# moss-lab/ScanFold

Hardware: AMD Instinct MI355X
Metric: windows/sec (W=120, step=1, 100 shuffles) (higher is better)
Workload: dtype int32 (int16 LDS storage) energies; f64 partition function

## Files before the change

scanfold_amd/csrc/scanfold_hip.hip:

```cpp
#include <math.h>
#include <stddef.h>
#include <stdio.h>
#include <stdlib.h>
#include <string.h>

#include <algorithm>
#include <map>
#include <string>
#include <vector>

#include "../../include/scanfold_hip_long.h"
#include "sf_launch.h"
#include "sf_energy.h"
#include "sf_mfe_full.hip.h"
#include "sf_mfe_fast.hip.h"
#include "sf_mfe_long.hip.h"
#include "sf_mfe_long_batch.hip.h"
#include "sf_mfe_banded.hip.h"
#include "sf_mfe_banded_batch.hip.h"
#include "sf_pf.hip.h"
#include "sf_pf_long.hip.h"
#include "sf_pf_long_batch.hip.h"
#include "sf_pf_banded.hip.h"
#include "sf_pf_fast.hip.h"
// ... 584 lines not shown
    g.slot[k].src.assign((const unsigned char *)&P, (const unsigned char *)&P + nb);
    if (blob_37c) {
      g.slot[k].src.insert(g.slot[k].src.end(), (const unsigned char *)&P37, (const unsigned char *)&P37 + nb);
      g.slot[k].src.insert(g.slot[k].src.end(), (const unsigned char *)&PdH, (const unsigned char *)&PdH + nb);
    }
    g.slot[k].key = key; g.slot[k].valid = true; g.slot[k].fast_ok = F.fast_ok; g.slot[k].span = g.max_bp_span;
    g.slot[k].temperature = temperature_c;
    g.slot[k].pf_kT = X.kT; g.slot[k].pf_MLbase = X.MLbase; g.slot[k].pf_hp30 = X.hp_init[30];
    hit = k;
  } else if (g.slot[hit].span != g.max_bp_span) {
    HIPCHK(hipDeviceSynchronize());
    HIPCHK(hipMemcpy((char *)g.slot[hit].dP + offsetof(SfDevParams, max_pair_dist), &md, sizeof md, hipMemcpyHostToDevice));
    g.slot[hit].span = g.max_bp_span;
  }
  g.slot[hit].used = g.loads;
  g.cur = hit;
  g.dP = g.slot[hit].dP; g.dX = g.slot[hit].dX; g.dF = g.slot[hit].dF;
  g.fast_ok = g.slot[hit].fast_ok;
  g.temperature = temperature_c;
  g.have_params = true;
  return SF_OK;
}

int sf_mfe_batch_dev(const uint8_t *d_seqs, int n, int W, int32_t *d_out, void *stream) {
  int rc = check_ready();
  if (rc) return rc;
  if (n < 0 || W < 1 || W > SF_MAX_W || (n > 0 && (!d_seqs || !d_out))) return SF_ERR_BAD_ARG;
  return launch_mfe(d_seqs, n, W, d_out, stream ? (hipStream_t)stream : g.stream);
}

int sf_mfe_batch(const uint8_t *seqs, int n, int W, int32_t *out) {
  int rc = check_ready();
  if (rc) return rc;
  if (n < 0 || W < 1 || W > SF_MAX_W || (n > 0 && (!seqs || !out))) return SF_ERR_BAD_ARG;
  if (n == 0) return SF_OK;
  if ((rc = ensure(g.seqs, (size_t)n * W))) return rc;
  if ((rc = ensure(g.energies, (size_t)n * sizeof(int32_t)))) return rc;
  HIPCHK(hipMemcpyAsync(g.seqs.p, seqs, (size_t)n * W, hipMemcpyHostToDevice, g.stream));
  if ((rc = launch_mfe((const uint8_t *)g.seqs.p, n, W, (int32_t *)g.energies.p, g.stream))) return rc;
  HIPCHK(hipMemcpyAsync(out, g.energies.p, (size_t)n * sizeof(int32_t), hipMemcpyDeviceToHost, g.stream));
  HIPCHK(hipStreamSynchronize(g.stream));
  return SF_OK;
}

int sf_mfe_trace_batch(const uint8_t *seqs, int n, int W, int32_t *mfe_out, char *db_out) {
  int rc = check_ready();
  if (rc) return rc;
  if (n < 0 || W < 1 || W > SF_MAX_W || (n > 0 && (!seqs || !db_out))) return SF_ERR_BAD_ARG;
  if (n == 0) return SF_OK;
  if ((rc = ensure(g.seqs, (size_t)n * W))) return rc;
  if ((rc = ensure(g.energies, (size_t)n * sizeof(int32_t)))) return rc;
  if ((rc = ensure(g.db, (size_t)n * (W + 1)))) return rc;
  HIPCHK(hipMemcpyAsync(g.seqs.p, seqs, (size_t)n * W, hipMemcpyHostToDevice, g.stream));
  if ((rc = launch_mfe((const uint8_t *)g.seqs.p, n, W, (int32_t *)g.energies.p, g.stream, 1, (char *)g.db.p)))
    return rc;
  if (mfe_out)
    HIPCHK(hipMemcpyAsync(mfe_out, g.energies.p, (size_t)n * sizeof(int32_t), hipMemcpyDeviceToHost, g.stream));
  HIPCHK(hipMemcpyAsync(db_out, g.db.p, (size_t)n * (W + 1), hipMemcpyDeviceToHost, g.stream));
  return read_status(g.stream, false);
}

int sf_pf_batch(const uint8_t *seqs, int n, int W, double *ens_dG, double *mbd, char *centroid, double *cdist) {
  int rc = check_ready();
  if (rc) return rc;
  if (n < 0 || W < 1 || W > SF_MAX_W || (n > 0 && !seqs)) return SF_ERR_BAD_ARG;
  if (n == 0) return SF_OK;
  if ((rc = ensure(g.seqs, (size_t)n * W))) return rc;
  if ((rc = ensure(g.dbl, (size_t)n * 3 * sizeof(double)))) return rc;
  if ((rc = ensure(g.cen, (size_t)n * (W + 1)))) return rc;
  double *d_dG = (double *)g.dbl.p, *d_mbd = d_dG + n, *d_cd = d_mbd + n;
  HIPCHK(hipMemcpyAsync(g.seqs.p, seqs, (size_t)n * W, hipMemcpyHostToDevice, g.stream));
  if ((rc = launch_pf((const uint8_t *)g.seqs.p, n, 1, W, d_dG, d_mbd, (char *)g.cen.p, d_cd, g.stream))) return rc;
  if ((rc = pf_results_to_host(n, W, ens_dG, mbd, centroid, cdist))) return rc;
  HIPCHK(hipStreamSynchronize(g.stream));
  return SF_OK;
}

static int scan_constraints(const uint8_t *seqs, const char *cons, int n, int W, bool *noncanonical) {
  static const uint8_t can[5][5] = {{0, 0, 0, 0, 0}, {0, 0, 0, 0, 1}, {0, 0, 0, 1, 0}, {0, 0, 1, 0, 1}, {0, 1, 0, 1, 0}};
  std::vector<int> stack((size_t)W + 1);
  *noncanonical = false;
  for (int k = 0; k < n; k++) {
    const char *c = cons + (size_t)k * W;
    const uint8_t *s = seqs + (size_t)k * W;
    int sp = 0;
    for (int i = 0; i < W; i++) {
      if (c[i] == '(') stack[sp++] = i;
      else if (c[i] == ')') {
        if (sp == 0) return SF_ERR_CONSTRAINT;
        const int o = stack[--sp];
        if (!can[sf_encode_nt(s[o])][sf_encode_nt(s[i])]) *noncanonical = true;
      }
    }
    if (sp) return SF_ERR_CONSTRAINT;
  }
  return SF_OK;
}

int sf_fold_constrained(const uint8_t *seqs, int n, int W, const char *cons, const int32_t *sc_stack_dcal, unsigned flags,
                        int32_t *mfe_out, char *db_out, double *ens_dG, double *mbd, char *centroid, double *cdist) {
  int rc = check_ready();
  if (rc) return rc;
  if (n < 0 || W < 1 || W > SF_MAX_W || (n > 0 && !seqs)) return SF_ERR_BAD_ARG;
  if (n == 0) return SF_OK;
  const bool want_mfe = !(flags & SF_FOLD_NO_MFE), want_pf = !(flags & SF_FOLD_NO_PF);
  bool noncanonical = false;
  if (cons && (rc = scan_constraints(seqs, cons, n, W, &noncanonical))) return rc;
  if ((rc = ensure(g.seqs, (size_t)n * W))) return rc;
  HIPCHK(hipMemcpyAsync(g.seqs.p, seqs, (size_t)n * W, hipMemcpyHostToDevice, g.stream));
  const char *d_cons = nullptr;
  const int32_t *d_sc = nullptr;
  if (cons) {
    if ((rc = ensure(g.cons, (size_t)n * W))) return rc;
    HIPCHK(hipMemcpyAsync(g.cons.p, cons, (size_t)n * W, hipMemcpyHostToDevice, g.stream));
    d_cons = (const char *)g.cons.p;
  }
  if (sc_stack_dcal) {
    if ((rc = ensure(g.sc, (size_t)n * W * sizeof(int32_t)))) return rc;
    HIPCHK(hipMemcpyAsync(g.sc.p, sc_stack_dcal, (size_t)n * W * sizeof(int32_t), hipMemcpyHostToDevice, g.stream));
    d_sc = (const int32_t *)g.sc.p;
  }
  if (want_mfe) {
    if ((rc = ensure(g.energies, (size_t)n * sizeof(int32_t)))) return rc;
    if ((rc = ensure(g.db, (size_t)n * (W + 1)))) return rc;
    rc = launch_mfe((const uint8_t *)g.seqs.p, n, W, (int32_t *)g.energies.p, g.stream, 1, (char *)g.db.p, d_cons, d_sc, noncanonical);
    if (rc) return rc;
    if (mfe_out)
      HIPCHK(hipMemcpyAsync(mfe_out, g.energies.p, (size_t)n * sizeof(int32_t), hipMemcpyDeviceToHost, g.stream));
    if (db_out) HIPCHK(hipMemcpyAsync(db_out, g.db.p, (size_t)n * (W + 1), hipMemcpyDeviceToHost, g.stream));
  }
  if (want_pf) {
    if ((rc = ensure(g.dbl, (size_t)n * 3 * sizeof(double)))) return rc;
    if ((rc = ensure(g.cen, (size_t)n * (W + 1)))) return rc;
    double *d_dG = (double *)g.dbl.p, *d_mbd = d_dG + n, *d_cd = d_mbd + n;
    if ((rc = launch_pf((const uint8_t *)g.seqs.p, n, 1, W, d_dG, d_mbd, (char *)g.cen.p, d_cd, g.stream, d_cons, noncanonical)))
      return rc;
    if ((rc = pf_results_to_host(n, W, ens_dG, mbd, centroid, cdist))) return rc;
  }
  return read_status(g.stream, false);
}

static int check_scan_args(int L, int W, int step, int win_begin, int n_win, int r, int kind) {
  if (L < 1 || W < 1 || W > SF_MAX_W || step < 1 || win_begin < 0 || n_win < 0 || r < 0) return SF_ERR_BAD_ARG;
  if (kind != SF_SHUFFLE_MONO && kind != SF_SHUFFLE_DI) return SF_ERR_BAD_ARG;
  if (n_win > 0 && (long long)(win_begin + n_win - 1) * step + W > L) return SF_ERR_BAD_ARG;
  return SF_OK;
}

static int launch_shuffle(const uint8_t *d_tr, int L, int W, int step, int win_begin, int n_win, int r, int kind,
                          uint64_t seed, uint8_t *d_seqs, hipStream_t st) {
  const long long total = (long long)n_win * (r + 1);
  if (total <= 0) return SF_OK;
  const int grid = (int)((total + SF_SHUF_BLOCK - 1) / SF_SHUF_BLOCK);
  SF_LAUNCH(sf_shuffle_kernel, grid, SF_SHUF_BLOCK, sf_shuffle_lds_bytes(W), st, d_tr, L, W, step, win_begin, n_win, r, kind, seed, d_seqs);
  HIPCHK(hipGetLastError());
  return SF_OK;
}

int sf_shuffle_windows(const uint8_t *transcript, int L, int W, int step, int win_begin, int n_win, int r, int kind,
                       uint64_t seed, uint8_t *seqs_out) {
  SF_ENTER();
  int rc = check_scan_args(L, W, step, win_begin, n_win, r, kind);
  if (rc) return rc;
  if (!transcript || (n_win > 0 && !seqs_out)) return SF_ERR_BAD_ARG;
  if (n_win == 0) return SF_OK;
  const size_t nb = (size_t)n_win * (r + 1) * W;
  if ((rc = ensure(g.transcript, (size_t)L))) return rc;
  if ((rc = ensure(g.seqs, nb))) return rc;
  HIPCHK(hipMemcpyAsync(g.transcript.p, transcript, (size_t)L, hipMemcpyHostToDevice, g.stream));
  if ((rc = launch_shuffle((const uint8_t *)g.transcript.p, L, W, step, win_begin, n_win, r, kind, seed,
                           (uint8_t *)g.seqs.p, g.stream)))
    return rc;
  HIPCHK(hipMemcpyAsync(seqs_out, g.seqs.p, nb, hipMemcpyDeviceToHost, g.stream));
  HIPCHK(hipStreamSynchronize(g.stream));
  return SF_OK;
}

int sf_scan_dev(const uint8_t *d_tr, int L, int W, int step, int win_begin, int n_win, int r, int kind, uint64_t seed,
                unsigned flags, int32_t *d_energies, char *d_structure, char *d_centroid, double *d_ens_div,
                double *d_ens_dG, void *stream) {
  int rc = check_ready();
  if (rc) return rc;
  if ((rc = check_scan_args(L, W, step, win_begin, n_win, r, kind))) return rc;
  if (!d_tr || (n_win > 0 && !d_energies)) return SF_ERR_BAD_ARG;
  if (n_win == 0) return SF_OK;
  hipStream_t st = stream ? (hipStream_t)stream : g.stream;
  const size_t row_bytes = (size_t)(r + 1) * W;
  int chunk = (int)(((size_t)1 << 30) / row_bytes);
  if (chunk < 1) chunk = 1;
  if (chunk > n_win) chunk = n_win;
  if ((rc = ensure(g.seqs, (size_t)chunk * row_bytes))) return rc;
  uint8_t *d_seqs = (uint8_t *)g.seqs.p;
  for (int w0 = 0; w0 < n_win; w0 += chunk) {
    const int nw = (n_win - w0 < chunk) ? n_win - w0 : chunk;
    if ((rc = launch_shuffle(d_tr, L, W, step, win_begin + w0, nw, r, kind, seed, d_seqs, st))) return rc;
    char *dbp = (!(flags & SF_SCAN_NO_TRACE) && d_structure) ? d_structure + (size_t)w0 * (W + 1) : nullptr;
    if ((rc = launch_mfe(d_seqs, nw * (r + 1), W, d_energies + (size_t)w0 * (r + 1), st, r + 1, dbp))) return rc;
    if (!(flags & SF_SCAN_NO_PF)) {
      if ((rc = launch_pf(d_seqs, nw, r + 1, W, d_ens_dG ? d_ens_dG + w0 : nullptr, d_ens_div ? d_ens_div + w0 : nullptr,
                          d_centroid ? d_centroid + (size_t)w0 * (W + 1) : nullptr, nullptr, st, nullptr, false,
                          d_tr, L, win_begin + w0, step)))
        return rc;
    }
  }
  return SF_OK;
}

int sf_scan(const uint8_t *transcript, int L, int W, int step, int win_begin, int n_win, int r, int kind, uint64_t seed,
            unsigned flags, int32_t *energies, char *structure, char *centroid, double *ens_div, double *ens_dG) {
  int rc = check_ready();
  if (rc) return rc;
  if ((rc = check_scan_args(L, W, step, win_begin, n_win, r, kind))) return rc;
  if (!transcript || (n_win > 0 && !energies)) return SF_ERR_BAD_ARG;
  if (n_win == 0) return SF_OK;
  const size_t ne = (size_t)n_win * (r + 1);
  if ((rc = ensure(g.transcript, (size_t)L))) return rc;
  if ((rc = ensure(g.energies, ne * sizeof(int32_t)))) return rc;
  if ((rc = ensure(g.db, (size_t)n_win * (W + 1)))) return rc;
  if ((rc = ensure(g.cen, (size_t)n_win * (W + 1)))) return rc;
  if ((rc = ensure(g.dbl, (size_t)n_win * 2 * sizeof(double)))) return rc;
  double *d_div = (double *)g.dbl.p, *d_dG = d_div + n_win;
  HIPCHK(hipMemcpyAsync(g.transcript.p, transcript, (size_t)L, hipMemcpyHostToDevice, g.stream));
  rc = sf_scan_dev((const uint8_t *)g.transcript.p, L, W, step, win_begin, n_win, r, kind, seed, flags,
                   (int32_t *)g.energies.p, structure ? (char *)g.db.p : nullptr, centroid ? (char *)g.cen.p : nullptr,
                   ens_div ? d_div : nullptr, ens_dG ? d_dG : nullptr, g.stream);
  if (rc) return rc;
  HIPCHK(hipMemcpyAsync(energies, g.energies.p, ne * sizeof(int32_t), hipMemcpyDeviceToHost, g.stream));
  if (structure && !(flags & SF_SCAN_NO_TRACE))
    HIPCHK(hipMemcpyAsync(structure, g.db.p, (size_t)n_win * (W + 1), hipMemcpyDeviceToHost, g.stream));
  if (!(flags & SF_SCAN_NO_PF)) {
    if (centroid) HIPCHK(hipMemcpyAsync(centroid, g.cen.p, (size_t)n_win * (W + 1), hipMemcpyDeviceToHost, g.stream));
    if (ens_div) HIPCHK(hipMemcpyAsync(ens_div, d_div, n_win * sizeof(double), hipMemcpyDeviceToHost, g.stream));
    if (ens_dG) HIPCHK(hipMemcpyAsync(ens_dG, d_dG, n_win * sizeof(double), hipMemcpyDeviceToHost, g.stream));
  }
  return read_status(g.stream, false);
}

struct TabOut {
  int32_t *gk, *gj, *gcount, *gfirst;
  double *sz, *sm, *se;
};
static TabOut tab_out_views(int64_t n) {
  TabOut o;
  char *p = (char *)g.tab_out.p;
  const size_t n8 = ((size_t)n + 1) & ~(size_t)1;
  o.gk = (int32_t *)p;
  o.gj = o.gk + n8;
  o.gcount = o.gj + n8;
  o.gfirst = o.gcount + n8;
  o.sz = (double *)(o.gfirst + n8);
  o.sm = o.sz + n8;
  o.se = o.sm + n8;
  return o;
}

int sf_tabulate_pairs(const char *structures, int row_stride, int structures_on_device, int n_win, int W,
                      const int32_t *starts, const double *z, const double *mfe, const double *ed, int64_t *n_groups) {
  SF_ENTER();
  g.tab_groups = -1;
  if (n_win < 1 || W < 1 || W > SF_MAX_W || row_stride < W || !structures || !starts || !z || !mfe || !ed || !n_groups)
    return SF_ERR_BAD_ARG;
  for (int w = 1; w < n_win; w++)
    if (starts[w] <= starts[w - 1]) return SF_ERR_TABLE;
  const int64_t span = (int64_t)starts[n_win - 1] + W - starts[0];
  if (span > 0x7fffff00 || (int64_t)n_win * W > 0x7fffff00) return SF_ERR_BAD_ARG;
  const int lo = starts[0], n_coords = (int)span;
  hipStream_t st = g.stream;
  const size_t off_z = (((size_t)n_win * 4) + 7) & ~(size_t)7;
  const size_t off_s = off_z + 3 * (size_t)n_win * 8;
  int rc = ensure(g.tab_in, off_s + (structures_on_device ? 0 : (size_t)n_win * row_stride));
  if (rc) return rc;
  char *in = (char *)g.tab_in.p;
  HIPCHK(hipMemcpyAsync(in, starts, (size_t)n_win * 4, hipMemcpyHostToDevice, st));
  HIPCHK(hipMemcpyAsync(in + off_z, z, (size_t)n_win * 8, hipMemcpyHostToDevice, st));
  HIPCHK(hipMemcpyAsync(in + off_z + (size_t)n_win * 8, mfe, (size_t)n_win * 8, hipMemcpyHostToDevice, st));
  HIPCHK(hipMemcpyAsync(in + off_z + 2 * (size_t)n_win * 8, ed, (size_t)n_win * 8, hipMemcpyHostToDevice, st));
  const char *d_structs = structures;
  if (!structures_on_device) {
    HIPCHK(hipMemcpyAsync(in + off_s, structures, (size_t)n_win * row_stride, hipMemcpyHostToDevice, st));
    d_structs = in + off_s;
  } else {
    HIPCHK(hipDeviceSynchronize());
  }
  const int32_t *d_starts = (const int32_t *)in;
  const double *d_z = (const double *)(in + off_z), *d_m = d_z + n_win, *d_e = d_m + n_win;
  rc = ensure(g.tab_partner, (size_t)n_win * W * sizeof(int16_t));
  if (rc) return rc;
  rc = ensure(g.tab_counts, ((size_t)n_coords + 1) * sizeof(int32_t));
  if (rc) return rc;
  int16_t *d_partner = (int16_t *)g.tab_partner.p;
  int32_t *d_counts = (int32_t *)g.tab_counts.p;
  int *d_status = (int *)g.status.p;
  SF_LAUNCH(sf_tab_partner_kernel, (n_win + 63) / 64, 64, (size_t)64 * (W / 2 + 1) * sizeof(int16_t), st, d_structs,
            row_stride, n_win, W, d_partner, d_status);
  SF_LAUNCH(sf_tab_groups_kernel<false>, n_coords, 64, 0, st, (const int16_t *)d_partner, d_starts, n_win, W, lo, d_counts,
            d_z, d_m, d_e, (int32_t *)nullptr, (int32_t *)nullptr, (int32_t *)nullptr, (int32_t *)nullptr,
            (double *)nullptr, (double *)nullptr, (double *)nullptr, d_status);
  SF_LAUNCH(sf_tab_scan_kernel, 1, 256, 0, st, d_counts, n_coords);
  HIPCHK(hipGetLastError());
  int32_t total = 0;
  HIPCHK(hipMemcpyAsync(&total, d_counts + n_coords, sizeof total, hipMemcpyDeviceToHost, st));
  rc = read_status(st, false);
  if (rc) return rc;
  const size_t n8 = ((size_t)total + 1) & ~(size_t)1;
  rc = ensure(g.tab_out, n8 * (4 * sizeof(int32_t) + 3 * sizeof(double)) + 16);
  if (rc) return rc;
  TabOut o = tab_out_views(total);
// ... 1248 lines not shown
  A.s1 = d1; A.s2 = d2; A.len1 = dl1; A.len2 = dl2; A.n = n; A.ld = ld;
  if ((rc = launch_duplex_batch(B, A, max1, max2))) return rc;
  HIPCHK(hipMemcpyAsync(energy_out, A.e, n * sizeof(int32_t), hipMemcpyDeviceToHost, g.stream));
  if (i_out) HIPCHK(hipMemcpyAsync(i_out, A.i, n * sizeof(int32_t), hipMemcpyDeviceToHost, g.stream));
  if (j_out) HIPCHK(hipMemcpyAsync(j_out, A.j, n * sizeof(int32_t), hipMemcpyDeviceToHost, g.stream));
  if (structure_out)
    HIPCHK(hipMemcpyAsync(structure_out, A.structure, (size_t)n * SF_DUPLEX_STRUCT_LEN, hipMemcpyDeviceToHost, g.stream));
  return read_status(g.stream, false);
}

int sf_lri_grid(int L, int kmer, int step, int32_t *n_j, int32_t *n_k) {
  if (L < 0 || kmer < 2 || step < 1 || !n_j || !n_k) return SF_ERR_BAD_ARG;
  int a, b;
  lri_grid(L, kmer, step, &a, &b);
  *n_j = a; *n_k = b;
  return SF_OK;
}

int sf_lri_scan(const uint8_t *seq, int L, int kmer, int step, int32_t cutoff_dcal, int64_t max_hits, sf_lri_hit *hits_out,
                int64_t *n_hits_out, int32_t *dense_e, int32_t *dense_i, int32_t *dense_j) {
  int rc = check_ready();
  if (rc) return rc;
  const bool dense = dense_e != nullptr;
  if (!seq || L < 1 || kmer < 2 || kmer > SF_DUPLEX_MAX_LEN || step < 1 || max_hits < 0 || max_hits > 0x7fffffffLL)
    return SF_ERR_BAD_ARG;
  if (dense ? (!dense_i || !dense_j) : (!n_hits_out || (max_hits > 0 && !hits_out))) return SF_ERR_BAD_ARG;
  if (n_hits_out) *n_hits_out = 0;
  int n_j, n_k;
  lri_grid(L, kmer, step, &n_j, &n_k);
  g_lri_ms = 0.0;
  g_lri_duplexes = 0;
  if (n_j == 0 || n_k == 0) return SF_OK;
  if (dense && (long long)n_j * n_k > 0x7fffffffLL / 4) return SF_ERR_BAD_ARG;

  std::vector<uint8_t> codes((size_t)L);
  for (int x = 0; x < L; x++) codes[x] = sf_encode_nt(seq[x]);
  CallBufs B("sf_lri_scan");
  SfLriScan A;
  memset(&A, 0, sizeof A);
  uint8_t *dcodes;
  if ((rc = B.upload(&dcodes, codes.data(), codes.size(), "sequence"))) return rc;
  A.codes = dcodes; A.L = L; A.kmer = kmer; A.step = step; A.n_j = n_j; A.n_k = n_k;
  A.n_chunk = (n_k + SF_DUP_BLOCK - 1) / SF_DUP_BLOCK;
  A.cutoff = cutoff_dcal;
  A.max_hits = (unsigned)max_hits;
  const size_t nd = (size_t)n_j * n_k;
  if (dense) {
    if ((rc = B.alloc(&A.dense_e, nd, "dense energies")) || (rc = B.alloc(&A.dense_i, nd, "dense i")) ||
        (rc = B.alloc(&A.dense_j, nd, "dense j")))
      return rc;
  } else {
    if ((rc = B.alloc(&A.hits, (size_t)max_hits, "hits"))) return rc;
  }
  if ((rc = B.alloc(&A.n_hits, 1, "hit count"))) return rc;
  HIPCHK(hipMemsetAsync(A.n_hits, 0, sizeof(unsigned), g.stream));

  const long long tasks = (long long)n_j * A.n_chunk;
  const int grid = dup_grid(tasks);
  const size_t strands = (size_t)kmer * SF_DUP_BLOCK + (size_t)kmer;
  const size_t ctab = (size_t)kmer * kmer * SF_DUP_BLOCK * sizeof(int16_t);
  const bool ldsc = ctab + strands <= SF_DUP_LDS_BUDGET;
  const size_t lds = ldsc ? ctab + strands : strands;
  if (strands > SF_DUP_LDS_BUDGET) return SF_ERR_BAD_ARG;
  if (ldsc) {
    HIPCHK(hipFuncSetAttribute((const void *)sf_lri_scan_kernel<true>, hipFuncAttributeMaxDynamicSharedMemorySize, (int)lds));
  } else {
    if ((rc = B.alloc(&A.scratch, ctab / sizeof(int16_t) * grid, "duplex tables"))) return rc;
  }
  long long per_launch = (long long)(8.0e6 * (20.0 / kmer) * (20.0 / kmer) * (20.0 / kmer) * (20.0 / kmer)) / SF_DUP_BLOCK;
  if (per_launch < grid) per_launch = grid;
  for (int k = 0; k < 2; k++) HIPCHK(hipEventCreate(&B.ev[k]));
  HIPCHK(hipEventRecord(B.ev[0], g.stream));
  for (long long t0 = 0; t0 < tasks; t0 += per_launch) {
    const long long t1 = t0 + per_launch < tasks ? t0 + per_launch : tasks;
    if (ldsc)
      SF_LAUNCH(sf_lri_scan_kernel<true>, grid, SF_DUP_BLOCK, lds, g.stream, A, t0, t1, (const SfDevParams *)g.dP);
    else
      SF_LAUNCH(sf_lri_scan_kernel<false>, grid, SF_DUP_BLOCK, lds, g.stream, A, t0, t1, (const SfDevParams *)g.dP);
    HIPCHK(hipGetLastError());
  }
  HIPCHK(hipEventRecord(B.ev[1], g.stream));
  unsigned count = 0;
  HIPCHK(hipMemcpyAsync(&count, A.n_hits, sizeof count, hipMemcpyDeviceToHost, g.stream));
  HIPCHK(hipStreamSynchronize(g.stream));
  float ms = 0;
  HIPCHK(hipEventElapsedTime(&ms, B.ev[0], B.ev[1]));
  g_lri_ms = ms;
  {
    long long nd2 = 0;
    for (int jx = 0; jx < n_j; jx++) {
      const long long jw = (long long)jx * step;
      const long long lo = jw - kmer - 4;
      long long below = lo < 0 ? 0 : lo / step + 1;
      if (below > n_k) below = n_k;
      long long above = n_k - ((jw + kmer + 3) / step + 1);
      if (above < 0) above = 0;
      nd2 += below + above;
    }
    g_lri_duplexes = nd2;
  }
  if (dense) {
    HIPCHK(hipMemcpy(dense_e, A.dense_e, nd * sizeof(int32_t), hipMemcpyDeviceToHost));
    HIPCHK(hipMemcpy(dense_i, A.dense_i, nd * sizeof(int32_t), hipMemcpyDeviceToHost));
    HIPCHK(hipMemcpy(dense_j, A.dense_j, nd * sizeof(int32_t), hipMemcpyDeviceToHost));
    return SF_OK;
  }
  *n_hits_out = (int64_t)count;
  if ((int64_t)count > max_hits) return SF_ERR_DUPLEX_HITS;
  if (count) {
    std::vector<sf_lri_hit> h(count);
    HIPCHK(hipMemcpy(h.data(), A.hits, (size_t)count * sizeof(sf_lri_hit), hipMemcpyDeviceToHost));
    std::sort(h.begin(), h.end(), [](const sf_lri_hit &a, const sf_lri_hit &b) {
      return a.j_win != b.j_win ? a.j_win < b.j_win : a.k_win < b.k_win;
    });
    memcpy(hits_out, h.data(), (size_t)count * sizeof(sf_lri_hit));
  }
  return SF_OK;
}

int sf_lri_scan_time(double *ms, int64_t *duplexes) {
  SF_ENTER();
  if (ms) *ms = g_lri_ms;
  if (duplexes) *duplexes = g_lri_duplexes;
  return SF_OK;
}

int sf_lri_background(const uint8_t *seq, int L, int kmer, const int32_t *j_win, const int32_t *k_win, int n_hits, int r,
                      int kind, uint64_t seed, int32_t *energies_out, uint8_t *rows1_out, uint8_t *rows2_out) {
  int rc = check_ready();
  if (rc) return rc;
  if (!seq || L < 1 || kmer < 2 || kmer > SF_DUPLEX_MAX_LEN || n_hits < 0 || r < 0 || r > 0x3fffffff) return SF_ERR_BAD_ARG;
  if (kind != SF_SHUFFLE_MONO && kind != SF_SHUFFLE_DI) return SF_ERR_BAD_ARG;
  if (n_hits == 0) return SF_OK;
  if (!j_win || !k_win || !energies_out) return SF_ERR_BAD_ARG;
  const long long rows = (long long)n_hits * (r + 1);
  if (rows > 0x7fffffffLL / SF_DUPLEX_MAX_LEN) return SF_ERR_BAD_ARG;
  for (int h = 0; h < n_hits; h++)
    if (j_win[h] < 0 || j_win[h] > L - kmer + 1 || k_win[h] < 0 || k_win[h] > L - kmer) return SF_ERR_BAD_ARG;
  std::vector<uint8_t> codes((size_t)L);
  for (int x = 0; x < L; x++) codes[x] = sf_encode_nt(seq[x]);
  CallBufs B("sf_lri_background");
  uint8_t *dcodes, *r1, *r2;
  int32_t *djw, *dkw, *l1;
  if ((rc = B.upload(&dcodes, codes.data(), codes.size(), "sequence")) || (rc = B.upload(&djw, j_win, (size_t)n_hits, "j_win")) ||
      (rc = B.upload(&dkw, k_win, (size_t)n_hits, "k_win")))
    return rc;
  SfDupBatch A;
  memset(&A, 0, sizeof A);
  const size_t nb = (size_t)rows * kmer;
  if ((rc = B.alloc(&r1, nb, "first strands")) || (rc = B.alloc(&r2, nb, "second strands")) ||
      (rc = B.alloc(&l1, (size_t)rows, "lengths")) || (rc = B.alloc(&A.e, (size_t)rows, "energies")))
    return rc;
  const int sgrid = (int)((rows + SF_SHUF_BLOCK - 1) / SF_SHUF_BLOCK);
  SF_LAUNCH(sf_lri_shuffle_kernel, sgrid, SF_SHUF_BLOCK, sf_shuffle_lds_bytes(kmer), g.stream, (const uint8_t *)dcodes, L, kmer,
            (const int32_t *)djw, (const int32_t *)dkw, n_hits, r, kind, seed, r1, r2, l1);
  HIPCHK(hipGetLastError());
  A.s1 = r1; A.s2 = r2; A.len1 = l1; A.len2 = nullptr;
  A.n = (int)rows; A.ld = kmer; A.n2 = kmer;
  if ((rc = launch_duplex_batch(B, A, kmer, kmer))) return rc;
  HIPCHK(hipMemcpyAsync(energies_out, A.e, rows * sizeof(int32_t), hipMemcpyDeviceToHost, g.stream));
  if (rows1_out) HIPCHK(hipMemcpyAsync(rows1_out, r1, nb, hipMemcpyDeviceToHost, g.stream));
  if (rows2_out) HIPCHK(hipMemcpyAsync(rows2_out, r2, nb, hipMemcpyDeviceToHost, g.stream));
  return read_status(g.stream, false);
}

}
```

scanfold_amd/csrc/sf_shuffle.hip.h:

```cpp
#pragma once
#include "sf_energy.h"

struct SfPhilox {
  uint32_t k0, k1;
  uint32_t c0, c1, c2, c3;
  uint32_t out[4];
  int have;
};
__device__ __forceinline__ uint32_t sf_mulhi32(uint32_t a, uint32_t b) { return (uint32_t)(((uint64_t)a * b) >> 32); }
__device__ inline void sf_philox_block(SfPhilox *g) {
  uint32_t c0 = g->c0, c1 = g->c1, c2 = g->c2, c3 = g->c3, k0 = g->k0, k1 = g->k1;
  for (int r = 0; r < 10; r++) {
    const uint32_t hi0 = sf_mulhi32(0xD2511F53u, c0), lo0 = 0xD2511F53u * c0;
    const uint32_t hi1 = sf_mulhi32(0xCD9E8D57u, c2), lo1 = 0xCD9E8D57u * c2;
    const uint32_t n0 = hi1 ^ c1 ^ k0, n2 = hi0 ^ c3 ^ k1;
    c0 = n0; c1 = lo1; c2 = n2; c3 = lo0;
    k0 += 0x9E3779B9u; k1 += 0xBB67AE85u;
  }
  g->out[0] = c0; g->out[1] = c1; g->out[2] = c2; g->out[3] = c3;
  g->c0++;
  g->have = 4;
}
__device__ inline uint32_t sf_rand_u32(SfPhilox *g) {
  if (!g->have) sf_philox_block(g);
  return g->out[4 - g->have--];
}
__device__ inline double sf_rand_double(SfPhilox *g) {
  const uint32_t a = sf_rand_u32(g) >> 5, b = sf_rand_u32(g) >> 6;
  return ((double)a * 67108864.0 + (double)b) * (1.0 / 9007199254740992.0);
}

__device__ __forceinline__ void sf_shuffle_row(const uint8_t *src, int W, int kind, SfPhilox &g, uint8_t *out, uint8_t *lst,
                                               uint16_t *cnt) {
  if (kind == SF_SHUFFLE_MONO) {
    for (int x = 0; x < W; x++) out[x] = sf_encode_nt(src[x]);
    for (int i = W - 1; i >= 1; i--) {
      const int jj = (int)(((uint64_t)sf_rand_u32(&g) * (uint32_t)(i + 1)) >> 32);
      const uint8_t t = out[i]; out[i] = out[jj]; out[jj] = t;
    }
  } else {
    const int order[5] = {1, 2, 3, 4, 0};
    for (int x = 0; x < 25; x++) cnt[x] = 0;
    uint8_t prev = sf_encode_nt(src[0]);
    const uint8_t first = prev;
    for (int x = 1; x < W; x++) {
      const uint8_t y = sf_encode_nt(src[x]);
      cnt[prev * 5 + y]++;
      prev = y;
    }
    const int lastCh = prev;
    int outdeg[5], present[5], lastedge[5];
    for (int a = 0; a < 5; a++) {
      int s = 0;
      for (int b = 0; b < 5; b++) s += cnt[a * 5 + b];
      outdeg[a] = s;
      present[a] = (s > 0) || (a == lastCh);
    }
    for (;;) {
      for (int oa = 0; oa < 5; oa++) {
        const int a = order[oa];
        lastedge[a] = -1;
        if (!present[a] || a == lastCh) continue;
        const double z = sf_rand_double(&g);
        const double denom = (double)outdeg[a];
        int num = 0, pick = order[4];
        for (int ob = 0; ob < 4; ob++) {
          num += cnt[a * 5 + order[ob]];
          if (z < (double)num / denom) { pick = order[ob]; break; }
        }
        lastedge[a] = pick;
      }
      int Dm[5];
      for (int a = 0; a < 5; a++) Dm[a] = (lastedge[a] == lastCh);
      for (int rnd = 0; rnd < 4; rnd++)
        for (int oa = 0; oa < 5; oa++) {
          const int a = order[oa];
          if (lastedge[a] >= 0 && Dm[lastedge[a]]) Dm[a] = 1;
        }
      int ok = 1;
      for (int a = 0; a < 5; a++)
        if (present[a] && a != lastCh && !Dm[a]) ok = 0;
      if (ok) break;
    }
    int start[5], fill[5];
    {
      int acc = 0;
      for (int oa = 0; oa < 5; oa++) { const int a = order[oa]; start[a] = acc; acc += outdeg[a]; fill[a] = 0; }
    }
    prev = first;
    for (int x = 1; x < W; x++) {
      const uint8_t y = sf_encode_nt(src[x]);
      lst[start[prev] + fill[prev]++] = y;
      prev = y;
    }
    for (int oa = 0; oa < 5; oa++) {
      const int a = order[oa];
      if (lastedge[a] < 0) continue;
      uint8_t *Lx = lst + start[a];
      int pos = 0;
      while (Lx[pos] != (uint8_t)lastedge[a]) pos++;
      for (int x = pos; x + 1 < outdeg[a]; x++) Lx[x] = Lx[x + 1];
    }
    for (int oa = 0; oa < 5; oa++) {
      const int a = order[oa];
      if (!present[a]) continue;
      uint8_t *Lx = lst + start[a];
      const int nlist = outdeg[a] - (lastedge[a] >= 0 ? 1 : 0);
      int barrier = nlist;
      for (int x = 0; x < nlist - 1; x++) {
        const int z = (int)(sf_rand_double(&g) * (double)barrier);
        const uint8_t t = Lx[z]; Lx[z] = Lx[barrier - 1]; Lx[barrier - 1] = t;
        barrier--;
      }
      if (lastedge[a] >= 0) Lx[nlist] = (uint8_t)lastedge[a];
    }
    int ptr[5] = {0, 0, 0, 0, 0};
    out[0] = first;
    int pc = first;
    for (int x = 1; x < W - 1; x++) {
      const uint8_t ch = lst[start[pc] + ptr[pc]++];
      out[x] = ch;
      pc = ch;
    }
    if (W > 1) out[W - 1] = (uint8_t)lastCh;
  }
}

#define SF_SHUF_BLOCK 64

static inline size_t sf_shuffle_lds_bytes(int W) {
  return (((size_t)SF_SHUF_BLOCK * W + 3) & ~(size_t)3) * 2 + SF_SHUF_BLOCK * 25 * sizeof(uint16_t);
}
__global__ void sf_shuffle_kernel(const uint8_t *__restrict__ transcript, int L, int W, int step, int win_begin,
                                  int n_win, int r, int kind, uint64_t seed, uint8_t *__restrict__ seqs_out) {
  SF_DYN_SMEM(smem);
  uint8_t *rows = (uint8_t *)smem;
  uint8_t *lsts = rows + (size_t)SF_SHUF_BLOCK * W;
  uint16_t *cnts = (uint16_t *)(lsts + (((size_t)SF_SHUF_BLOCK * W + 3) & ~(size_t)3));
  const int lane = threadIdx.x;
  const long long total = (long long)n_win * (r + 1);
  const long long row0 = (long long)blockIdx.x * SF_SHUF_BLOCK;
  const long long row = row0 + lane;
  uint8_t *out = rows + (size_t)lane * W;
  uint8_t *lst = lsts + (size_t)lane * W;
  uint16_t *cnt = cnts + lane * 25;
  (void)L;

  if (row < total) {
    const int w = (int)(row / (r + 1)), k = (int)(row % (r + 1));
    const uint8_t *src = transcript + (size_t)(win_begin + w) * step;
    if (k == 0) {
      for (int x = 0; x < W; x++) out[x] = sf_encode_nt(src[x]);
    } else {
      SfPhilox g;
      g.k0 = (uint32_t)seed; g.k1 = (uint32_t)(seed >> 32);
      g.c0 = 0; g.c1 = (uint32_t)k; g.c2 = (uint32_t)(win_begin + w); g.c3 = (uint32_t)kind;
      g.have = 0;
      sf_shuffle_row(src, W, kind, g, out, lst, cnt);
    }
  }
  __syncthreads();
  long long nrows = total - row0;
  if (nrows > SF_SHUF_BLOCK) nrows = SF_SHUF_BLOCK;
  const size_t nbytes = (size_t)nrows * W;
  uint8_t *dst = seqs_out + (size_t)row0 * W;
  for (size_t x = lane; x < nbytes; x += SF_SHUF_BLOCK) dst[x] = rows[x];
}
```

Baseline: 44470.

## Restructure shuffle kernel with shared per-window staging and interleaved LDS lists

New measurement: 44770, median of 6. No clear change (+0.7%).

```diff
diff --git a/scanfold_amd/csrc/scanfold_hip.hip b/scanfold_amd/csrc/scanfold_hip.hip
--- a/scanfold_amd/csrc/scanfold_hip.hip
+++ b/scanfold_amd/csrc/scanfold_hip.hip
@@ -760,7 +760,7 @@
   const long long total = (long long)n_win * (r + 1);
   if (total <= 0) return SF_OK;
   const int grid = (int)((total + SF_SHUF_BLOCK - 1) / SF_SHUF_BLOCK);
-  SF_LAUNCH(sf_shuffle_kernel, grid, SF_SHUF_BLOCK, sf_shuffle_lds_bytes(W), st, d_tr, L, W, step, win_begin, n_win, r, kind, seed, d_seqs);
+  SF_LAUNCH(sf_shuffle_kernel, grid, SF_SHUF_BLOCK, sf_shuffle_lds_bytes(W, r), st, d_tr, L, W, step, win_begin, n_win, r, kind, seed, d_seqs);
   HIPCHK(hipGetLastError());
   return SF_OK;
 }
@@ -2315,7 +2315,7 @@
       (rc = B.alloc(&l1, (size_t)rows, "lengths")) || (rc = B.alloc(&A.e, (size_t)rows, "energies")))
     return rc;
   const int sgrid = (int)((rows + SF_SHUF_BLOCK - 1) / SF_SHUF_BLOCK);
-  SF_LAUNCH(sf_lri_shuffle_kernel, sgrid, SF_SHUF_BLOCK, sf_shuffle_lds_bytes(kmer), g.stream, (const uint8_t *)dcodes, L, kmer,
+  SF_LAUNCH(sf_lri_shuffle_kernel, sgrid, SF_SHUF_BLOCK, sf_shuffle_row_lds_bytes(kmer), g.stream, (const uint8_t *)dcodes, L, kmer,
             (const int32_t *)djw, (const int32_t *)dkw, n_hits, r, kind, seed, r1, r2, l1);
   HIPCHK(hipGetLastError());
   A.s1 = r1; A.s2 = r2; A.len1 = l1; A.len2 = nullptr;
diff --git a/scanfold_amd/csrc/sf_shuffle.hip.h b/scanfold_amd/csrc/sf_shuffle.hip.h
--- a/scanfold_amd/csrc/sf_shuffle.hip.h
+++ b/scanfold_amd/csrc/sf_shuffle.hip.h
@@ -23,146 +23,243 @@
 }
 __device__ inline uint32_t sf_rand_u32(SfPhilox *g) {
   if (!g->have) sf_philox_block(g);
-  return g->out[4 - g->have--];
+  const int at = 4 - g->have--;
+  return at == 0 ? g->out[0] : (at == 1 ? g->out[1] : (at == 2 ? g->out[2] : g->out[3]));
 }
 __device__ inline double sf_rand_double(SfPhilox *g) {
   const uint32_t a = sf_rand_u32(g) >> 5, b = sf_rand_u32(g) >> 6;
   return ((double)a * 67108864.0 + (double)b) * (1.0 / 9007199254740992.0);
 }
 
+#define SF_SHUF_FB 12
+__device__ __forceinline__ int sf_shuf_get(uint64_t p, int a) { return (int)(p >> (SF_SHUF_FB * a)) & ((1 << SF_SHUF_FB) - 1); }
+__device__ __forceinline__ uint64_t sf_shuf_one(int a) { return (uint64_t)1 << (SF_SHUF_FB * a); }
+
+template <class IO>
+__device__ __forceinline__ void sf_shuffle_core(IO &io, int W, int kind, SfPhilox &g) {
+  if (kind == SF_SHUFFLE_MONO) {
+    for (int x = 0; x < W; x++) io.lst(x) = io.src(x);
+    for (int i = W - 1; i >= 1; i--) {
+      const int jj = (int)(((uint64_t)sf_rand_u32(&g) * (uint32_t)(i + 1)) >> 32);
+      const uint8_t t = io.lst(i), u = io.lst(jj);
+      io.lst(i) = u; io.lst(jj) = t;
+    }
+    io.emit(W, [&](int x) { return io.lst(x); });
+    return;
+  }
+  constexpr int order[5] = {1, 2, 3, 4, 0};
+  const int first = io.src(0), lastCh = io.src(W - 1);
+  int outdeg[5];
+  unsigned present = 0;
+#pragma unroll
+  for (int a = 0; a < 5; a++) {
+    int s = 0;
+#pragma unroll
+    for (int b = 0; b < 5; b++) s += io.cnt(a, b);
+    outdeg[a] = s;
+    if (s > 0 || a == lastCh) present |= 1u << a;
+  }
+  unsigned lastedge;
+  for (;;) {
+    lastedge = 0x77777u;
+#pragma unroll
+    for (int oa = 0; oa < 5; oa++) {
+      const int a = order[oa];
+      if (!((present >> a) & 1) || a == lastCh) continue;
+      const double z = sf_rand_double(&g);
+      const double denom = (double)outdeg[a];
+      int num = 0, pick = order[4];
+#pragma unroll
+      for (int ob = 0; ob < 4; ob++) {
+        num += io.cnt(a, order[ob]);
+        if (z < (double)num / denom) { pick = order[ob]; break; }
+      }
+      lastedge = (lastedge & ~(0xfu << (4 * a))) | ((unsigned)pick << (4 * a));
+    }
+    unsigned Dm = 0;
+#pragma unroll
+    for (int a = 0; a < 5; a++)
+      if ((int)((lastedge >> (4 * a)) & 0xf) == lastCh) Dm |= 1u << a;
+    for (int rnd = 0; rnd < 4; rnd++)
+#pragma unroll
+      for (int oa = 0; oa < 5; oa++) {
+        const int a = order[oa];
+        const unsigned e = (lastedge >> (4 * a)) & 0xf;
+        if (e != 7 && ((Dm >> e) & 1)) Dm |= 1u << a;
+      }
+    if (!(present & ~(1u << lastCh) & ~Dm)) break;
+  }
+  uint64_t start = 0, nlist = 0;
+  {
+    int acc = 0;
+#pragma unroll
+    for (int oa = 0; oa < 5; oa++) {
+      const int a = order[oa];
+      start |= (uint64_t)acc << (SF_SHUF_FB * a);
+      nlist |= (uint64_t)(outdeg[a] - (((lastedge >> (4 * a)) & 0xf) != 7 ? 1 : 0)) << (SF_SHUF_FB * a);
+      acc += outdeg[a];
+    }
+  }
+  {
+    uint64_t cur = start;
+    unsigned pend = lastedge;
+    int prev = first;
+    for (int x = 1; x < W; x++) {
+      const int y = io.src(x);
+      const bool skip = (int)((pend >> (4 * prev)) & 0xf) == y;
+      if (skip) pend |= 7u << (4 * prev);
+      else {
+        io.lst(sf_shuf_get(cur, prev)) = (uint8_t)y;
+        cur += sf_shuf_one(prev);
+      }
+      prev = y;
+    }
+  }
+  {
+    int oa = -1, barrier = 0, base = 0;
+    for (;;) {
+      while (barrier < 2 && oa < 4) {
+        oa++;
+        const int a = oa == 4 ? 0 : oa + 1;
+        barrier = sf_shuf_get(nlist, a);
+        base = sf_shuf_get(start, a);
+      }
+      if (barrier < 2) break;
+      const int z = (int)(sf_rand_double(&g) * (double)barrier);
+      const uint8_t t = io.lst(base + z), u = io.lst(base + barrier - 1);
+      io.lst(base + z) = u; io.lst(base + barrier - 1) = t;
+      barrier--;
+    }
+#pragma unroll
+    for (int a = 0; a < 5; a++) {
+      const unsigned e = (lastedge >> (4 * a)) & 0xf;
+      if (e != 7) io.lst(sf_shuf_get(start, a) + sf_shuf_get(nlist, a)) = (uint8_t)e;
+    }
+  }
+  uint64_t ptr = start;
+  int pc = first;
+  io.emit(W, [&](int x) -> uint8_t {
+    if (x == 0) return (uint8_t)first;
+    if (x == W - 1) return (uint8_t)lastCh;
+    const uint8_t ch = io.lst(sf_shuf_get(ptr, pc));
+    ptr += sf_shuf_one(pc);
+    pc = ch;
+    return ch;
+  });
+}
+
+struct SfShufflePlain {
+  const uint8_t *s;
+  uint8_t *out, *l;
+  const uint16_t *c;
+  __device__ __forceinline__ int src(int x) const { return sf_encode_nt(s[x]); }
+  __device__ __forceinline__ int cnt(int a, int b) const { return c[a * 5 + b]; }
+  __device__ __forceinline__ uint8_t &lst(int x) { return l[x]; }
+  template <class F>
+  __device__ __forceinline__ void emit(int W, F f) {
+    for (int x = 0; x < W; x++) out[x] = f(x);
+  }
+};
 __device__ __forceinline__ void sf_shuffle_row(const uint8_t *src, int W, int kind, SfPhilox &g, uint8_t *out, uint8_t *lst,
                                                uint16_t *cnt) {
-  if (kind == SF_SHUFFLE_MONO) {
-    for (int x = 0; x < W; x++) out[x] = sf_encode_nt(src[x]);
-    for (int i = W - 1; i >= 1; i--) {
-      const int jj = (int)(((uint64_t)sf_rand_u32(&g) * (uint32_t)(i + 1)) >> 32);
-      const uint8_t t = out[i]; out[i] = out[jj]; out[jj] = t;
-    }
-  } else {
-    const int order[5] = {1, 2, 3, 4, 0};
+  if (kind != SF_SHUFFLE_MONO) {
     for (int x = 0; x < 25; x++) cnt[x] = 0;
     uint8_t prev = sf_encode_nt(src[0]);
-    const uint8_t first = prev;
     for (int x = 1; x < W; x++) {
       const uint8_t y = sf_encode_nt(src[x]);
       cnt[prev * 5 + y]++;
       prev = y;
     }
-    const int lastCh = prev;
-    int outdeg[5], present[5], lastedge[5];
-    for (int a = 0; a < 5; a++) {
-      int s = 0;
-      for (int b = 0; b < 5; b++) s += cnt[a * 5 + b];
-      outdeg[a] = s;
-      present[a] = (s > 0) || (a == lastCh);
-    }
-    for (;;) {
-      for (int oa = 0; oa < 5; oa++) {
-        const int a = order[oa];
-        lastedge[a] = -1;
-        if (!present[a] || a == lastCh) continue;
-        const double z = sf_rand_double(&g);
-        const double denom = (double)outdeg[a];
-        int num = 0, pick = order[4];
-        for (int ob = 0; ob < 4; ob++) {
-          num += cnt[a * 5 + order[ob]];
-          if (z < (double)num / denom) { pick = order[ob]; break; }
-        }
-        lastedge[a] = pick;
-      }
-      int Dm[5];
-      for (int a = 0; a < 5; a++) Dm[a] = (lastedge[a] == lastCh);
-      for (int rnd = 0; rnd < 4; rnd++)
-        for (int oa = 0; oa < 5; oa++) {
-          const int a = order[oa];
-          if (lastedge[a] >= 0 && Dm[lastedge[a]]) Dm[a] = 1;
-        }
-      int ok = 1;
-      for (int a = 0; a < 5; a++)
-        if (present[a] && a != lastCh && !Dm[a]) ok = 0;
-      if (ok) break;
-    }
-    int start[5], fill[5];
-    {
-      int acc = 0;
-      for (int oa = 0; oa < 5; oa++) { const int a = order[oa]; start[a] = acc; acc += outdeg[a]; fill[a] = 0; }
-    }
-    prev = first;
-    for (int x = 1; x < W; x++) {
-      const uint8_t y = sf_encode_nt(src[x]);
-      lst[start[prev] + fill[prev]++] = y;
-      prev = y;
-    }
-    for (int oa = 0; oa < 5; oa++) {
-      const int a = order[oa];
-      if (lastedge[a] < 0) continue;
-      uint8_t *Lx = lst + start[a];
-      int pos = 0;
-      while (Lx[pos] != (uint8_t)lastedge[a]) pos++;
-      for (int x = pos; x + 1 < outdeg[a]; x++) Lx[x] = Lx[x + 1];
-    }
-    for (int oa = 0; oa < 5; oa++) {
-      const int a = order[oa];
-      if (!present[a]) continue;
-      uint8_t *Lx = lst + start[a];
-      const int nlist = outdeg[a] - (lastedge[a] >= 0 ? 1 : 0);
-      int barrier = nlist;
-      for (int x = 0; x < nlist - 1; x++) {
-        const int z = (int)(sf_rand_double(&g) * (double)barrier);
-        const uint8_t t = Lx[z]; Lx[z] = Lx[barrier - 1]; Lx[barrier - 1] = t;
-        barrier--;
-      }
-      if (lastedge[a] >= 0) Lx[nlist] = (uint8_t)lastedge[a];
-    }
-    int ptr[5] = {0, 0, 0, 0, 0};
-    out[0] = first;
-    int pc = first;
-    for (int x = 1; x < W - 1; x++) {
-      const uint8_t ch = lst[start[pc] + ptr[pc]++];
-      out[x] = ch;
-      pc = ch;
-    }
-    if (W > 1) out[W - 1] = (uint8_t)lastCh;
-  }
+  }
+  SfShufflePlain io{src, out, lst, cnt};
+  sf_shuffle_core(io, W, kind, g);
 }
 
 #define SF_SHUF_BLOCK 64
 
-static inline size_t sf_shuffle_lds_bytes(int W) {
+static inline size_t sf_shuffle_row_lds_bytes(int W) {
   return (((size_t)SF_SHUF_BLOCK * W + 3) & ~(size_t)3) * 2 + SF_SHUF_BLOCK * 25 * sizeof(uint16_t);
 }
+
+__host__ __device__ static inline int sf_shuffle_block_windows(int r) {
+  const long long q = (SF_SHUF_BLOCK - 1) / ((long long)r + 1) + 2;
+  return q < SF_SHUF_BLOCK ? (int)q : SF_SHUF_BLOCK;
+}
+__host__ __device__ static inline size_t sf_shuffle_lst_bytes(int W) { return (size_t)((W + 3) / 4) * SF_SHUF_BLOCK * 4; }
+static inline size_t sf_shuffle_lds_bytes(int W, int r) {
+  return sf_shuffle_lst_bytes(W) + (size_t)sf_shuffle_block_windows(r) * (25 * sizeof(uint32_t) + W);
+}
+
+struct SfShuffleStaged {
+  const uint8_t *win;
+  const uint32_t *cw;
+  uint8_t *col;
+  uint8_t *dst;
+  __device__ __forceinline__ int src(int x) const { return win[x]; }
+  __device__ __forceinline__ int cnt(int a, int b) const { return (int)cw[a * 5 + b]; }
+  __device__ __forceinline__ uint8_t &lst(int x) { return col[((x >> 2) * SF_SHUF_BLOCK * 4) + (x & 3)]; }
+  template <class F>
+  __device__ __forceinline__ void emit(int W, F f) {
+    if (W & 3) {
+      for (int x = 0; x < W; x++) dst[x] = f(x);
+      return;
+    }
+    for (int x0 = 0; x0 < W; x0 += 16) {
+      uint32_t pk[4] = {0, 0, 0, 0};
+#pragma unroll
+      for (int t = 0; t < 16; t++)
+        if (x0 + t < W) pk[t >> 2] |= (uint32_t)f(x0 + t) << (8 * (t & 3));
+      uint32_t *d = (uint32_t *)__builtin_assume_aligned(dst + x0, 4);
+      if (x0 + 16 <= W) {
+        __builtin_memcpy(d, pk, 16);
+      } else {
+#pragma unroll
+        for (int q = 0; q < 3; q++)
+          if (x0 + 4 * q < W) d[q] = pk[q];
+      }
+    }
+  }
+};
+
 __global__ void sf_shuffle_kernel(const uint8_t *__restrict__ transcript, int L, int W, int step, int win_begin,
                                   int n_win, int r, int kind, uint64_t seed, uint8_t *__restrict__ seqs_out) {
   SF_DYN_SMEM(smem);
-  uint8_t *rows = (uint8_t *)smem;
-  uint8_t *lsts = rows + (size_t)SF_SHUF_BLOCK * W;
-  uint16_t *cnts = (uint16_t *)(lsts + (((size_t)SF_SHUF_BLOCK * W + 3) & ~(size_t)3));
+  const int nbw = sf_shuffle_block_windows(r);
+  uint8_t *lsts = (uint8_t *)smem;
+  uint32_t *cnts = (uint32_t *)(lsts + sf_shuffle_lst_bytes(W));
+  uint8_t *wins = (uint8_t *)(cnts + nbw * 25);
   const int lane = threadIdx.x;
   const long long total = (long long)n_win * (r + 1);
   const long long row0 = (long long)blockIdx.x * SF_SHUF_BLOCK;
   const long long row = row0 + lane;
-  uint8_t *out = rows + (size_t)lane * W;
-  uint8_t *lst = lsts + (size_t)lane * W;
-  uint16_t *cnt = cnts + lane * 25;
   (void)L;
 
-  if (row < total) {
-    const int w = (int)(row / (r + 1)), k = (int)(row % (r + 1));
-    const uint8_t *src = transcript + (size_t)(win_begin + w) * step;
-    if (k == 0) {
-      for (int x = 0; x < W; x++) out[x] = sf_encode_nt(src[x]);
-    } else {
-      SfPhilox g;
-      g.k0 = (uint32_t)seed; g.k1 = (uint32_t)(seed >> 32);
-      g.c0 = 0; g.c1 = (uint32_t)k; g.c2 = (uint32_t)(win_begin + w); g.c3 = (uint32_t)kind;
-      g.have = 0;
-      sf_shuffle_row(src, W, kind, g, out, lst, cnt);
-    }
+  long long rowl = row0 + SF_SHUF_BLOCK - 1;
+  if (rowl > total - 1) rowl = total - 1;
+  const int w0 = (int)(row0 / (r + 1)), nw = (int)(rowl / (r + 1)) - w0 + 1;
+  for (int x = lane; x < nw * 25; x += SF_SHUF_BLOCK) cnts[x] = 0;
+  for (int v = 0; v < nw; v++) {
+    const uint8_t *src = transcript + (size_t)(win_begin + w0 + v) * step;
+    for (int x = lane; x < W; x += SF_SHUF_BLOCK) wins[v * W + x] = sf_encode_nt(src[x]);
   }
   __syncthreads();
-  long long nrows = total - row0;
-  if (nrows > SF_SHUF_BLOCK) nrows = SF_SHUF_BLOCK;
-  const size_t nbytes = (size_t)nrows * W;
-  uint8_t *dst = seqs_out + (size_t)row0 * W;
-  for (size_t x = lane; x < nbytes; x += SF_SHUF_BLOCK) dst[x] = rows[x];
-}
+  if (kind != SF_SHUFFLE_MONO) {
+    for (int v = 0; v < nw; v++)
+      for (int x = lane + 1; x < W; x += SF_SHUF_BLOCK)
+        atomicAdd(&cnts[v * 25 + wins[v * W + x - 1] * 5 + wins[v * W + x]], 1u);
+    __syncthreads();
+  }
+  if (row >= total) return;
+
+  const int w = (int)(row / (r + 1)), k = (int)(row % (r + 1));
+  SfShuffleStaged io{wins + (w - w0) * W, cnts + (w - w0) * 25, lsts + lane * 4, seqs_out + (size_t)row * W};
+  if (k == 0) {
+    io.emit(W, [&](int x) { return (uint8_t)io.src(x); });
+  } else {
+    SfPhilox g;
+    g.k0 = (uint32_t)seed; g.k1 = (uint32_t)(seed >> 32);
+    g.c0 = 0; g.c1 = (uint32_t)k; g.c2 = (uint32_t)(win_begin + w); g.c3 = (uint32_t)kind;
+    g.have = 0;
+    sf_shuffle_core(io, W, kind, g);
+  }
+}
```
